# bioengstrom/tsbb15-3d-reconstruction-project

Measured on NVIDIA B200. Metric: f_ransac_evals_per_sec, higher is better.
Workload: dtype f32 scoring with f64 guard-band recheck; f64 solve

## Files before the change

include/rg_b200.h:

```cpp
#ifndef RG_B200_H
#define RG_B200_H

#include <stdint.h>

#ifdef __cplusplus
extern "C" {
#endif

#define RG_MODE_EPI_MAX 0
#define RG_MODE_SAMPSON 1
#define RG_TIE_FIRST 0
#define RG_TIE_REFERENCE 1
#define RG_SOLVER_QR 0
#define RG_SOLVER_JACOBI 1
#define RG_SCORE_FP32_GUARDED 0
#define RG_SCORE_FP64 1
#define RG_SCORE_FP32_BOUND 2

int rg_abi_version(void);
const char* rg_last_error(void);
int rg_init(int device, void** out_ctx);
int rg_shutdown(void* ctx);
int rg_device_sm_count(void* ctx);
int rg_host_alloc(size_t bytes, void** out);
int rg_host_free(void* p);
int rg_set_option(void* ctx, int option, long long value);
int rg_get_profile(void* ctx, void* stream, double* out_ms5, int* out_calls);

int rg_microbench_run(double* out6, void* stream);

int rg_get_last_stats(void* ctx, void* stream, long long* out8);

int rg_f_ransac_dev(void* ctx, void* stream, int P, const double* pts64_dev, const int32_t* pair_off_host,
                    const int32_t* idx_dev, const int32_t* hyp_off_host, double thr, int mode, int tie_mode, int solver,
                    int score_path, int32_t* best_idx_dev, int32_t* best_count_dev, double* best_F_dev,
                    unsigned char* mask_dev );
#define RG_FLAG_REUSE_POINTS 1
#define RG_FLAG_BOUNDED 2
int rg_f_ransac_dev2(void* ctx, void* stream, int P, const double* pts64_dev, const int32_t* pair_off_host,
                     const int32_t* idx_dev , const int32_t* hyp_off_host, double thr, int mode,
                     int tie_mode, int solver, int score_path, int flags, unsigned long long sample_seed, int first_pair_id,
                     int hyp_index_base, int32_t* best_idx_dev, int32_t* best_count_dev, double* best_F_dev,
                     unsigned char* mask_dev , unsigned long long* key_dev );
int rg_sample_indices_dev(void* ctx, void* stream, int P, const int32_t* n_points_host, const int32_t* hyp_off_host, int k,
                          unsigned long long seed, int first_pair_id, int hyp_index_base, int32_t* idx_out_dev);
int rg_synth_two_view_dev(void* ctx, void* stream, int P, int first_pair_id, int N, const double* cams_host, int n_cams,
                          const double* bbox6_host, unsigned long long seed_base, double outlier_frac, double sigma_px,
                          double width, double height, double* pts_out_dev, int32_t* cam_pair_out_dev);
int rg_f_inlier_mask_dev(void* ctx, void* stream, int P, const double* pts64_dev, const int32_t* pair_off_host,
                         const double* F_dev, double thr, int mode, unsigned char* mask_dev);
int rg_f_last_hypotheses_dev(void* ctx, const int32_t** counts_dev, const double** F_all_dev,
                             const unsigned char** flags_dev);
int rg_f_last_bounded_stats(void* ctx, void* stream, long long* out4);
int rg_f_last_bounded_evals(void* ctx, void* stream, long long* out2);
int rg_f_ransac_host(void* ctx, void* stream, int P, const double* pts64, const int32_t* pair_off, const int32_t* idx,
                     const int32_t* hyp_off, double thr, int mode, int tie_mode, int solver, int score_path,
                     int32_t* best_idx, int32_t* best_count, double* best_F, unsigned char* mask, int32_t* counts,
                     double* F_all, unsigned char* flags);

int rg_f_ransac_host2(void* ctx, void* stream, int P, const double* pts64, const int32_t* pair_off,
                      const int32_t* idx , const int32_t* hyp_off, double thr, int mode, int tie_mode,
                      int solver, int score_path, unsigned long long sample_seed, int first_pair_id, int32_t* best_idx,
                      int32_t* best_count, double* best_F, unsigned char* mask, int32_t* counts, double* F_all,
                      unsigned char* flags);

int rg_f8pt_solve_host(void* ctx, void* stream, int N, const double* pts64, int H, const int32_t* idx, int solver,
                       double* F_all, unsigned char* flags );
int rg_epi_score_count_host(void* ctx, void* stream, int N, const double* pts64, int H, const double* F_all, double thr,
                            int mode, int score_path, int32_t* counts);
int rg_fmatrix_residuals_host(void* ctx, void* stream, const double* F9, int N, const double* x, const double* y,
// ... 91 lines not shown
```

tsbb15-3d-reconstruction-project_b200/_cabi.py:

```python
from __future__ import annotations

import ctypes as C
import os
import threading

import numpy as np

_HERE = os.path.dirname(os.path.abspath(__file__))
LIB_PATH = os.environ.get("RG_LIB", os.path.join(_HERE, "librg_b200.so"))

MODE_EPI_MAX, MODE_SAMPSON = 0, 1
TIE_FIRST, TIE_REFERENCE = 0, 1
SOLVER_QR, SOLVER_JACOBI = 0, 1
SCORE_FP32_GUARDED, SCORE_FP64, SCORE_FP32_BOUND = 0, 1, 2
TRI_OPTIMAL, TRI_LINEAR = 0, 1
FLAG_REUSE_POINTS = 1
FLAG_BOUNDED = 2

_vp = C.c_void_p
_i = C.c_int
_d = C.c_double
_pd = C.POINTER(C.c_double)
_pll = C.POINTER(C.c_longlong)

SIGNATURES = {
    "rg_abi_version": (_i, []),
    "rg_last_error": (C.c_char_p, []),
    "rg_init": (_i, [_i, C.POINTER(_vp)]),
    "rg_shutdown": (_i, [_vp]),
    "rg_device_sm_count": (_i, [_vp]),
    "rg_host_alloc": (_i, [C.c_size_t, C.POINTER(_vp)]),
    "rg_host_free": (_i, [_vp]),
    "rg_set_option": (_i, [_vp, _i, C.c_longlong]),
    "rg_get_profile": (_i, [_vp, _vp, _pd, C.POINTER(C.c_int)]),
    "rg_microbench_run": (_i, [_pd, _vp]),
    "rg_get_last_stats": (_i, [_vp, _vp, _pll]),
    "rg_f_ransac_dev": (_i, [_vp, _vp, _i, _vp, _vp, _vp, _vp, _d, _i, _i, _i, _i, _vp, _vp, _vp, _vp]),
    "rg_f_ransac_dev2": (_i, [_vp, _vp, _i, _vp, _vp, _vp, _vp, _d, _i, _i, _i, _i, _i, C.c_ulonglong, _i, _i, _vp, _vp, _vp, _vp, _vp]),
    "rg_f_ransac_host2": (_i, [_vp, _vp, _i, _vp, _vp, _vp, _vp, _d, _i, _i, _i, _i, C.c_ulonglong, _i, _vp, _vp, _vp, _vp, _vp, _vp, _vp]),
    "rg_sample_indices_dev": (_i, [_vp, _vp, _i, _vp, _vp, _i, C.c_ulonglong, _i, _i, _vp]),
    "rg_synth_two_view_dev": (_i, [_vp, _vp, _i, _i, _i, _vp, _i, _vp, C.c_ulonglong, _d, _d, _d, _d, _vp, _vp]),
    "rg_f_inlier_mask_dev": (_i, [_vp, _vp, _i, _vp, _vp, _vp, _d, _i, _vp]),
    "rg_pnp_ransac_batched_dev2": (_i, [_vp, _vp, _i, _vp, _vp, _vp, _vp, _vp, _vp, _i, _d, _i, _i, _vp, _vp, _vp, _vp, _vp]),
    "rg_p2p_create": (_i, [_vp, _i, _i, _vp]),
    "rg_p2p_connect": (_i, [_vp, _vp]),
    "rg_p2p_destroy": (_i, [_vp]),
    "rg_p2p_argmax_exchange": (_i, [_vp, _vp, _i, _vp, _vp, _i, _vp, _vp, _vp, _vp]),
    "rg_f_last_hypotheses_dev": (_i, [_vp, C.POINTER(_vp), C.POINTER(_vp), C.POINTER(_vp)]),
    "rg_f_last_bounded_stats": (_i, [_vp, _vp, _pll]),
    "rg_f_last_bounded_evals": (_i, [_vp, _vp, _pll]),
    "rg_f_ransac_host": (_i, [_vp, _vp, _i, _vp, _vp, _vp, _vp, _d, _i, _i, _i, _i, _vp, _vp, _vp, _vp, _vp, _vp, _vp]),
    "rg_f8pt_solve_host": (_i, [_vp, _vp, _i, _vp, _i, _vp, _i, _vp, _vp]),
    "rg_epi_score_count_host": (_i, [_vp, _vp, _i, _vp, _i, _vp, _d, _i, _i, _vp]),
    "rg_fmatrix_residuals_host": (_i, [_vp, _vp, _vp, _i, _vp, _vp, _vp]),
    "rg_fmatrix_stls_host": (_i, [_vp, _vp, _i, _vp, _vp, _vp]),
    "rg_pnp_ransac_host": (_i, [_vp, _vp, _i, _i, _vp, _vp, _i, _i, _vp, _d, _i, _vp, _vp, _vp, _vp, _vp, _vp, _vp, _vp]),
    "rg_pnp_ransac_dev": (_i, [_vp, _vp, _i, _i, _vp, _vp, _i, _i, _vp, _d, _i, _vp, _vp, _vp, _vp]),
    "rg_pnp_ransac_batched_host": (_i, [_vp, _vp, _i, _vp, _vp, _vp, _vp, _vp, _vp, _i, _d, _i, _vp, _vp, _vp, _vp, _vp, _vp, _vp]),
    "rg_pnp_ransac_batched_dev": (_i, [_vp, _vp, _i, _vp, _vp, _vp, _vp, _vp, _vp, _i, _d, _i, _vp, _vp, _vp, _vp]),
    "rg_pnp_minimize_host": (_i, [_vp, _vp, _i, _vp, _vp, _vp, _vp]),
    "rg_pnp_score_count_host": (_i, [_vp, _vp, _i, _vp, _vp, _i, _vp, _d, _i, _vp]),
    "rg_triangulate_host": (_i, [_vp, _vp, _i, _vp, _vp, _vp, _vp, _vp, _i, _vp]),
    "rg_triangulate_dev": (_i, [_vp, _vp, _i, _vp, _vp, _vp, _vp, _vp, _i, _vp]),
    "rg_fmatrix_from_cameras_host": (_i, [_vp, _vp, _i, _vp, _vp, _vp]),
    "rg_relative_pose_host": (_i, [_vp, _vp, _i, _vp, _vp, _i, _vp, _vp, _vp, _vp, _vp]),
    "rg_relative_pose_dev": (_i, [_vp, _vp, _i, _vp, _vp, _i, _vp, _vp, _vp, _vp, _vp]),
    "rg_camera_resectioning_host": (_i, [_vp, _vp, _i, _vp, _vp, _vp, _vp]),
# ... 123 lines not shown
```

tsbb15-3d-reconstruction-project_b200/build.py:

```python
import os
import subprocess
import sys

HERE = os.path.dirname(os.path.abspath(__file__))
CSRC = os.path.join(HERE, "csrc")
LIB = os.path.join(HERE, "librg_b200.so")
SOURCES = ["librg_b200.cu"]
HEADERS = ["ctx.cu", "f_api.cu", "pnp_api.cu", "geom_api.cu", "geom_kernels.cuh", "gs_api.cu", "gs_kernels.cuh", "ba_api.cu", "ba_kernels.cuh", "nccl_api.cu", "p2p_api.cu", "philox.cuh", "microbench.cu", "common.cuh", "score_core.cuh", "f_kernels.cuh", "jacobi.cuh", "pnp_kernels.cuh", "pnp_refine_api.cu", "pnp_refine_kernels.cuh", "tall.cuh", "plan.cuh", "bounded.cuh"]
NVCC_FLAGS = ["-gencode", "arch=compute_100a,code=sm_100a", "-lineinfo", "-O3", "-std=c++17",
              "-Xcompiler", "-fPIC", "-shared", "-Xptxas", "-v", "-ldl"]


def _stale() -> bool:
    if not os.path.isfile(LIB):
        return True
    t = os.path.getmtime(LIB)
    for f in SOURCES + HEADERS:
        p = os.path.join(CSRC, f)
        if os.path.isfile(p) and os.path.getmtime(p) > t:
            return True
    return os.path.getmtime(os.path.abspath(__file__)) > t


LIB_DEBUG = os.path.join(HERE, "librg_b200_debug.so")


def build_debug(force: bool = False) -> str:
    if not force and os.path.isfile(LIB_DEBUG) and os.path.getmtime(LIB_DEBUG) >= max(
            os.path.getmtime(os.path.join(CSRC, f)) for f in SOURCES + HEADERS if os.path.isfile(os.path.join(CSRC, f))):
        return LIB_DEBUG
    nvcc = os.environ.get("NVCC", "/usr/local/cuda/bin/nvcc")
    flags = [f for f in NVCC_FLAGS if f not in ("-Xptxas", "-v")]
    cmd = [nvcc] + flags + ["-DRG_DEBUG"] + [os.path.join(CSRC, f) for f in SOURCES] + ["-o", LIB_DEBUG]
    res = subprocess.run(cmd, capture_output=True, text=True)
    if res.returncode != 0:
        sys.stderr.write(res.stdout + res.stderr)
        raise RuntimeError("nvcc failed building librg_b200_debug.so")
    return LIB_DEBUG


def build(force: bool = False, verbose: bool = False) -> str:
    if not force and not _stale():
        return LIB
    nvcc = os.environ.get("NVCC", "/usr/local/cuda/bin/nvcc")
    srcs = [os.path.join(CSRC, f) for f in SOURCES if os.path.isfile(os.path.join(CSRC, f))]
    cmd = [nvcc] + NVCC_FLAGS + srcs + ["-o", LIB]
    res = subprocess.run(cmd, capture_output=True, text=True)
    if verbose or res.returncode != 0:
        sys.stderr.write(res.stdout + res.stderr)
    if res.returncode != 0:
        raise RuntimeError("nvcc failed building librg_b200.so")
    with open(os.path.join(HERE, "build_ptxas.log"), "w") as f:
        f.write(res.stdout + res.stderr)
    return LIB


if __name__ == "__main__":
    print(build(force="--force" in sys.argv, verbose=True))
    if "--debug" in sys.argv:
        print(build_debug(force="--force" in sys.argv))
```

tsbb15-3d-reconstruction-project_b200/csrc/common.cuh:

```cuda
#pragma once
#include <cuda_runtime.h>
#include <cstdint>
#include <cstddef>
#include <cstdio>
#include <cstring>
#include <cmath>
#include <vector>
#ifdef RG_DEBUG
#include <cassert>
#define RG_ASSERT(cond) assert(cond)
#else
#define RG_ASSERT(cond) ((void)0)
#endif

namespace rg {

enum : int {
    RG_OK = 0,
    RG_ERR_CUDA = -1,
    RG_ERR_ARG = -2,
    RG_ERR_NO_DEVICE = -3,
};

void set_error(const char* fmt, ...);

#define RG_CUDA(call)                                                                       \
    do {                                                                                    \
        cudaError_t _e = (call);                                                            \
        if (_e != cudaSuccess) {                                                            \
            ::rg::set_error("%s:%d: %s -> %s", __FILE__, __LINE__, #call, cudaGetErrorString(_e)); \
            return ::rg::RG_ERR_CUDA;                                                       \
        }                                                                                   \
    } while (0)

#define RG_CHECK_ARG(cond, msg)                                   \
    do {                                                          \
        if (!(cond)) {                                            \
            ::rg::set_error("invalid argument: %s", msg);         \
            return ::rg::RG_ERR_ARG;                              \
        }                                                         \
    } while (0)

enum : int { MODE_EPI_MAX = 0, MODE_SAMPSON = 1 };
enum : int { TIE_FIRST = 0, TIE_REFERENCE = 1 };
enum : int { SOLVER_QR = 0, SOLVER_JACOBI = 1 };
enum : int { SCORE_FP32_GUARDED = 0, SCORE_FP64 = 1, SCORE_FP32_BOUND = 2 };

struct __align__(16) Hyp32 {
    float f[9];
    float g[5];
    float G;
    float T;
};
static_assert(sizeof(Hyp32) == 64, "Hyp32 layout");

struct __align__(16) Pose32 {
    float p[12];
    float G;
    float pad0, pad1, pad2;
};
static_assert(sizeof(Pose32) == 64, "Pose32 layout");

constexpr int kSub = 8;

__device__ __forceinline__ int find_segment(const int* __restrict__ off, int P, int i) {
    int lo = 0, hi = P;
    while (hi - lo > 1) {
        int mid = (lo + hi) >> 1;
        if (off[mid] <= i) lo = mid; else hi = mid;
    }
    return lo;
}

__device__ __forceinline__ uint32_t smem_u32(const void* p) {
    return (uint32_t)__cvta_generic_to_shared(p);
}

__device__ __forceinline__ void mbar_init(uint64_t* bar, uint32_t count) {
    asm volatile("mbarrier.init.shared::cta.b64 [%0], %1;" ::"r"(smem_u32(bar)), "r"(count));
}
__device__ __forceinline__ void fence_mbar_init() {
    asm volatile("fence.mbarrier_init.release.cluster;" ::: "memory");
}
__device__ __forceinline__ void fence_proxy_async() {
    asm volatile("fence.proxy.async.shared::cta;" ::: "memory");
}
__device__ __forceinline__ void mbar_expect_tx(uint64_t* bar, uint32_t bytes) {
    asm volatile("mbarrier.arrive.expect_tx.shared::cta.b64 _, [%0], %1;" ::"r"(smem_u32(bar)), "r"(bytes)
                 : "memory");
}
__device__ __forceinline__ bool mbar_try_wait(uint64_t* bar, uint32_t parity) {
    uint32_t ok;
    asm volatile(
        "{\n"
        ".reg .pred p;\n"
        "mbarrier.try_wait.parity.shared::cta.b64 p, [%1], %2;\n"
        "selp.u32 %0, 1, 0, p;\n"
        "}\n"
        : "=r"(ok)
// ... 35 lines not shown
    double c1x, c1y, c2x, c2y;
    double thr, B;
    double band_scale;
    double pad;
};

struct FPlan {
    int P = 0;
    long long Ntot = 0, Htot = 0, N32tot = 0;
    int n_items = 0;
    int maxN = 0, maxH = 0;
    double evals = 0.0;
    bool bounded = false;
    bool bound_prefix = false;
    int K = 0;
    long long Ctot = 0;
    int n_items_c = 0, n_items_f = 0;
    double evals_c = 0.0, evals_f = 0.0;
};

struct Ctx {
    int device = 0;
    int sm_count = 0;
    Buffer pair_info, pair_frame, state, pts32, F64, hyp32, flags, flag_list, stats, best, tie_stats, bbox;
    Buffer bnd;
    int* counts_ptr = nullptr;
    unsigned char* ovf_ptr = nullptr;
    Buffer gen_idx;
    struct PassSet { Buffer pair_info, pair_frame, state, pts32, F64, hyp32, flags, flag_list, best, tie_stats, bnd; } spare[3];
    cudaStream_t tail_stream = nullptr;
    cudaEvent_t head_done[3] = {nullptr, nullptr, nullptr};
    cudaEvent_t score_done[3] = {nullptr, nullptr, nullptr};
    cudaEvent_t cand_done[3] = {nullptr, nullptr, nullptr};
    cudaEvent_t sweep_done[3] = {nullptr, nullptr, nullptr};
    cudaEvent_t tail_done[2] = {nullptr, nullptr};
    cudaEvent_t pipe_gate = nullptr;
    bool tail_pending[2] = {false, false};
    int tail_carve_max = -1;
    int ws_slot = 0;
    int opt_pipeline = 1;
    const void* prep_pts = nullptr; int prep_P = 0; long long prep_N = 0; double prep_thr = 0.0; unsigned long long prep_hash = 0;
    int last_passes = 0;
    double rate_evals_per_s = 0.0, rate_h2d_bytes_per_s = 0.0;
    cudaEvent_t rate_ev[4] = {nullptr, nullptr, nullptr, nullptr};
    bool pnp_rows_attr_set = false;
    int opt_pnp_solver = 0;
    long long opt_list_cap = 0;
    double opt_band_scale = 1.0;
    long long opt_pass_evals = 0;
    int opt_bounded = 1;
    int opt_rho_milli = 450;
    int opt_bounded_k = 512;
    int opt_bound_prefix = 1;
    bool last_bounded = false;
    long long bnd_host_evals = 0;
    long long bnd_bound_evals = 0;
    Buffer bnd_stats;
    void* p2p_local = nullptr; size_t p2p_bytes = 0; int p2p_rank = 0, p2p_world = 0; unsigned p2p_seq = 0;
    void* p2p_peer[16] = {nullptr};

    Buffer d_in_a, d_in_b, d_in_c;
    Buffer d_out_a, d_out_b, d_out_c, d_out_d;
    Buffer pose64, pose32, X32;
    Buffer geom;
    Buffer geom_ws;
    Buffer gs_ws;
    Buffer ba_ws;
    int opt_ba_cluster = 0;
    int opt_gs_multi = 0;
    int opt_ba_l2 = 0;
    Buffer pr_ws;
    int opt_pr_multi = 0;
    Buffer h_pr_flags;
    cudaEvent_t pr_iter_ev[2] = {nullptr, nullptr};
    Buffer h_ba_items;
    Buffer h_ba_flags;
    cudaEvent_t ba_iter_ev[2] = {nullptr, nullptr};
    bool ba_attr_set = false;
    Buffer h_stage[2], h_stats;
    cudaEvent_t staging_free[2] = {nullptr, nullptr};
    int stage_turn = 0;
    FPlan plan_cached; unsigned long long plan_hash = 0; const void* plan_table = nullptr; bool plan_valid = false;
    static constexpr int kMaxSlices = 8;
    cudaStream_t copy_stream = nullptr;
    std::vector<cudaEvent_t> pass_ready;
    std::vector<cudaEvent_t> pass_done;
    cudaStream_t d2h_stream = nullptr;
    cudaEvent_t d2h_done = nullptr;
    cudaEvent_t copy_gate = nullptr;
    int opt_host_slices = 0;
    bool accumulate_stats = false;
    long long last_stats[8] = {0, 0, 0, 0, 0, 0, 0, 0};
    int opt_profile = 0;
    static constexpr int kProfPhases = 5;
    static constexpr int kProfScoreStart = 6;
    static constexpr int kProfSweep = 7;
    static constexpr int kProfEvents = 11;
    static constexpr int kProfRing = 2048;
    cudaEvent_t* prof_ev = nullptr;
    int prof_cur = -1;
    int prof_calls = 0;
    bool prof_open = false;
    unsigned prof_masks[kProfRing] = {0};
};

int ensure_pinned(Buffer& b, size_t bytes);
// ... 10 lines not shown
```

tsbb15-3d-reconstruction-project_b200/csrc/ctx.cu:

```cuda
#include "common.cuh"
#include <cstdarg>
#include <mutex>

namespace rg {

static thread_local char g_err[1024] = "";

void set_error(const char* fmt, ...) {
    va_list ap;
    va_start(ap, fmt);
    vsnprintf(g_err, sizeof(g_err), fmt, ap);
    va_end(ap);
}

int ensure(Buffer& b, size_t bytes) {
    if (bytes <= b.cap) return RG_OK;
    size_t want = bytes + bytes / 4 + 256;
    if (b.ptr) {
        RG_CUDA(cudaFree(b.ptr));
        b.ptr = nullptr;
        b.cap = 0;
    }
    RG_CUDA(cudaMalloc(&b.ptr, want));
    b.cap = want;
// ... 182 lines not shown
        c->opt_ba_l2 = value != 0;
        return RG_OK;
    }
    if (option == 5) {
        c->opt_gs_multi = value != 0;
        return RG_OK;
    }
    if (option == 6) {
        if (value < 0) { set_error("invalid argument: option 6 (evaluations per pass) must be >= 0"); return RG_ERR_ARG; }
        c->opt_pass_evals = value;
        return RG_OK;
    }
    if (option == 7) {
        if (value != 0 && value != 1) { set_error("invalid argument: option 7 (PnP minimal solver) must be 0 or 1"); return RG_ERR_ARG; }
        c->opt_pnp_solver = (int)value;
        return RG_OK;
    }
    if (option == 9) {
        if (value < 1000 || value > 100000000ll) { set_error("invalid argument: option 9 (guard-band factor x 1000) must be in [1000, 1e8]"); return RG_ERR_ARG; }
        c->opt_band_scale = (double)value / 1000.0;
        c->prep_pts = nullptr;
        return RG_OK;
    }
    if (option == 10) {
        if (value != 0 && value != 1) { set_error("invalid argument: option 10 (pass pipelining) must be 0 or 1"); return RG_ERR_ARG; }
        c->opt_pipeline = (int)value;
        return RG_OK;
    }
    if (option == 11) {
        if (value != 0 && value != 1) { set_error("invalid argument: option 11 (PnP refinement path) must be 0 or 1"); return RG_ERR_ARG; }
        c->opt_pr_multi = (int)value;
        return RG_OK;
    }
    if (option == 12) {
        if (value != 0 && value != 1) { set_error("invalid argument: option 12 (bounded sweep) must be 0 or 1"); return RG_ERR_ARG; }
        c->opt_bounded = (int)value;
        return RG_OK;
    }
    if (option == 13) {
        if (value < 1 || value > 1000) { set_error("invalid argument: option 13 (prefix share x 1000) must be in [1, 1000]"); return RG_ERR_ARG; }
        c->opt_rho_milli = (int)value;
        return RG_OK;
    }
    if (option == 14) {
        if (value < 1 || value > 65536) { set_error("invalid argument: option 14 (candidates per pair) must be in [1, 65536]"); return RG_ERR_ARG; }
        c->opt_bounded_k = (int)value;
        return RG_OK;
    }
    if (option == 15) {
        if (value != 0 && value != 1) { set_error("invalid argument: option 15 (bound-only prefix stage) must be 0 or 1"); return RG_ERR_ARG; }
        c->opt_bound_prefix = (int)value;
        return RG_OK;
    }
    if (option == 8) {
        if (value < 0 || value > 1000000000ll) { set_error("invalid argument: option 8 (flag list capacity) must be in [0, 1e9]"); return RG_ERR_ARG; }
        c->opt_list_cap = value;
        return RG_OK;
    }
    set_error("invalid argument: unknown option %d", option);
    return RG_ERR_ARG;
}

int rg_get_profile(void* ctx, void* stream, double* out_ms5, int* out_calls) {
    RG_CHECK_ARG(ctx != nullptr && out_ms5 != nullptr && out_calls != nullptr, "null argument");
    Ctx* c = (Ctx*)ctx;
    RG_CUDA(cudaSetDevice(c->device));
    RG_CUDA(cudaStreamSynchronize((cudaStream_t)stream));
    for (int k = 0; k < Ctx::kProfPhases; ++k) out_ms5[k] = 0.0;
    *out_calls = c->prof_calls;
    int complete = 0;
    for (int call = 0; call < c->prof_calls; ++call) {
        const unsigned need = (1u << (Ctx::kProfPhases + 1)) - 1u;
        if ((c->prof_masks[call] & need) != need) continue;
        cudaEvent_t* e = c->prof_ev + call * Ctx::kProfEvents;
        const bool own_start = (c->prof_masks[call] >> Ctx::kProfScoreStart) & 1u;
        for (int k = 0; k < Ctx::kProfPhases; ++k) {
            float ms = 0.f;
            RG_CUDA(cudaEventElapsedTime(&ms, (k == 2 && own_start) ? e[Ctx::kProfScoreStart] : e[k], e[k + 1]));
            out_ms5[k] += ms;
        }
        for (int b = Ctx::kProfSweep; b + 1 < Ctx::kProfEvents; b += 2) {
            if (((c->prof_masks[call] >> b) & 3u) != 3u) continue;
            float ms = 0.f;
            RG_CUDA(cudaEventElapsedTime(&ms, e[b], e[b + 1]));
            out_ms5[2] += ms;
        }
        ++complete;
    }
    *out_calls = complete;
    c->prof_calls = 0;
    c->prof_open = false;
    c->prof_cur = -1;
    return RG_OK;
}

}
```

tsbb15-3d-reconstruction-project_b200/csrc/f_api.cu:

```cuda
#include "f_kernels.cuh"
#include "bounded.cuh"
#include "jacobi.cuh"
#include "philox.cuh"
#include "plan.cuh"
#include <algorithm>
#include <vector>

namespace rg {

enum : int { FLAG_REUSE_POINTS = 1, FLAG_BOUNDED = 2 };

constexpr double kDefaultPassEvals = 2.7e10;
constexpr long long kMaxPassHyp = 1ll << 22;

struct ScoreState {
    unsigned* bbox; int* counts; int* work; unsigned* list_n; unsigned char* ovf;
    size_t off_counts, bytes;
    int *c_work, *f_work, *f_items, *sfx_c, *sfx_f, *mark;
    unsigned *c_list_n, *f_list_n;
    unsigned char *ovf_c, *ovf_f;
};

int score_state_layout(Ctx* c, int P, long long Htot, int bbox_words, ScoreState& s, long long Ctot = -1) {
    const size_t H = (size_t)std::max<long long>(Htot, 1);
    const size_t bbox_bytes = (((size_t)std::max(P, 1) * bbox_words * 4) + 15) / 16 * 16;
    const size_t cnt_bytes = ((H + 2) * 4 + 15) / 16 * 16;
    const size_t ovf_bytes = (H + 15) / 16 * 16;
    const size_t C = (size_t)std::max<long long>(Ctot, 1);
    const size_t bnd_ints = Ctot >= 0 ? ((8 + C + H + (size_t)std::max(P, 1)) * 4 + 15) / 16 * 16 : 0;
    const size_t bnd_ovf = Ctot >= 0 ? (C + H + 15) / 16 * 16 : 0;
    s.off_counts = bbox_bytes;
    s.bytes = bbox_bytes + cnt_bytes + ovf_bytes + bnd_ints + bnd_ovf;
    int rc = ensure(c->state, s.bytes);
    if (rc) return rc;
    char* base = (char*)c->state.ptr;
    s.bbox = (unsigned*)base;
    s.counts = (int*)(base + bbox_bytes);
    s.work = s.counts + H;
    s.list_n = (unsigned*)(s.counts + H + 1);
    s.ovf = (unsigned char*)(base + bbox_bytes + cnt_bytes);
    if (Ctot >= 0) {
        int* b = (int*)(base + bbox_bytes + cnt_bytes + ovf_bytes);
        s.c_work = b; s.c_list_n = (unsigned*)(b + 1); s.f_work = b + 2; s.f_list_n = (unsigned*)(b + 3); s.f_items = b + 4;
        s.sfx_c = b + 8; s.sfx_f = s.sfx_c + C; s.mark = s.sfx_f + H;
        s.ovf_c = (unsigned char*)(base + bbox_bytes + cnt_bytes + ovf_bytes + bnd_ints);
        s.ovf_f = s.ovf_c + C;
    }
    c->counts_ptr = s.counts;
    c->ovf_ptr = s.ovf;
    return RG_OK;
}

struct BndWs { Hyp32* hypc; int* map; int4* sel; PairInfo* fb; };
static int bnd_workspace(Ctx* c, const FPlan& plan, BndWs& w) {
// ... 137 lines not shown

template <int MODE>
static int f_solve_launch(Ctx* c, cudaStream_t st, const FPlan& plan, const double* pts64, const int* idx, int solver,
                          unsigned long long seed = 0, unsigned first_pair = 0) {
    const PairInfo* pi = (const PairInfo*)c->pair_info.ptr;
    const PairFrame* fr = (const PairFrame*)c->pair_frame.ptr;
    if (plan.Htot == 0) return RG_OK;
    if (solver == SOLVER_QR) {
        f8_solve_qr<MODE><<<ceil_div(plan.Htot, 128), 128, 0, st>>>((const double4*)pts64, idx, seed, first_pair, pi, fr, plan.P,
                                                                  (int)plan.Htot, (double*)c->F64.ptr, (Hyp32*)c->hyp32.ptr,
                                                                  (unsigned char*)c->flags.ptr);
    } else {
        const int groups_per_block = kJacobiThreads / 16;
        f8_solve_jacobi<MODE><<<ceil_div(plan.Htot, groups_per_block), kJacobiThreads, 0, st>>>(
            (const double4*)pts64, idx, seed, first_pair, pi, fr, plan.P, (int)plan.Htot, (double*)c->F64.ptr,
            (Hyp32*)c->hyp32.ptr, (unsigned char*)c->flags.ptr);
    }
    c->last_stats[7] += 1;
    RG_CUDA(cudaGetLastError());
    return RG_OK;
}

struct PassCtl {
    FCall a;
    std::vector<int> po, ho;
    FPlan plan;
    ScoreState s;
    FlagList fl{nullptr, nullptr, 0u, nullptr};
    FlagList flc{nullptr, nullptr, 0u, nullptr}, flf{nullptr, nullptr, 0u, nullptr};
    BndWs bw{};
    bool scored = false;
    int slot = 0;
    int prof_call = -1;
    cudaEvent_t ready = nullptr;
    cudaEvent_t done = nullptr;
    cudaStream_t out_stream = nullptr; void* out_dst = nullptr; const void* out_src = nullptr; size_t out_bytes = 0;
};

template <int MODE>
static int f_score_only(Ctx* c, cudaStream_t st, PassCtl& k) {
    const FPlan& plan = k.plan;
    const PairInfo* pi = (const PairInfo*)c->pair_info.ptr;
    k.scored = false;
    if (plan.Htot == 0 || plan.Ntot == 0 || (k.a.score_path != SCORE_FP64 && plan.n_items == 0)) return RG_OK;
    if (k.a.score_path != SCORE_FP64) {
        int bps = 1, rc = score_blocks_per_sm<EpiPolicy<MODE>>(&bps);
        if (rc) return rc;
        k.fl = flag_list_for(c, k.s, std::max(plan.evals, plan.evals_f), &rc);
        if (rc) return rc;
        if (plan.bounded) {
            k.flc = FlagList{k.fl.rec, k.s.c_list_n, k.fl.cap, k.s.ovf_c};
            k.flf = FlagList{k.fl.rec, k.s.f_list_n, k.fl.cap, k.s.ovf_f};
        }
        if (plan.bound_prefix || k.a.score_path == SCORE_FP32_BOUND) {
            static_assert(score_smem_bytes<EpiBoundPolicy>() == score_smem_bytes<EpiPolicy<MODE>>(), "same stage ring");
            if ((rc = score_blocks_per_sm<EpiBoundPolicy>(&bps))) return rc;
            score_packed<EpiBoundPolicy><<<std::min(plan.n_items, c->sm_count * bps), kScoreThreads,
                                           score_smem_bytes<EpiBoundPolicy>(), st>>>(
                (const float4*)c->pts32.ptr, (const Hyp32*)c->hyp32.ptr, pi, plan.P, plan.n_items, k.s.counts, k.fl, k.s.work);
        } else {
            constexpr size_t smem = score_smem_bytes<EpiPolicy<MODE>>();
            const int grid = std::min(plan.n_items, c->sm_count * bps);
            score_packed<EpiPolicy<MODE>><<<grid, kScoreThreads, smem, st>>>((const float4*)c->pts32.ptr, (const Hyp32*)c->hyp32.ptr,
                                                                            pi, plan.P, plan.n_items, k.s.counts, k.fl, k.s.work);
        }
        k.scored = true;
    } else {
        const int zs = std::max(1, std::min(64, ceil_div(plan.maxN, 2048)));
        f_score_fp64<<<dim3(ceil_div(plan.maxH, 128), plan.P, zs), 128, 0, st>>>((const double4*)k.a.pts64, (const double*)c->F64.ptr,
                                                                                 pi, k.a.thr, MODE, k.s.counts);
    }
    c->last_stats[7] += 1;
    RG_CUDA(cudaGetLastError());
    return RG_OK;
}

enum : int { STAGE_MAIN = 0, STAGE_CAND = 1, STAGE_FALLBACK = 2 };
template <int MODE>
static int f_fixup_launch(Ctx* c, cudaStream_t ts, PassCtl& k, bool beside_scorer, int stage = STAGE_MAIN) {
    if (!k.scored) return RG_OK;
    const FPlan& plan = k.plan;
    const PairInfo* pi = (const PairInfo*)c->pair_info.ptr;
    const Hyp32* hyp = (const Hyp32*)c->hyp32.ptr;
    const int* map = nullptr;
    FlagList fl = k.fl;
    long long H = plan.Htot;
    int* counts = k.s.counts;
    double evals = plan.evals;
    if (stage == STAGE_CAND) {
        pi += plan.P; hyp = k.bw.hypc; map = k.bw.map; fl = k.flc; H = plan.Ctot; counts = k.s.sfx_c; evals = plan.evals_c;
    } else if (stage == STAGE_FALLBACK) {
        pi = k.bw.fb; fl = k.flf; counts = k.s.sfx_f; evals = plan.evals_f;
    }
    typename EpiFix<MODE>::Params fp{(const float4*)c->pts32.ptr, (const double4*)k.a.pts64, hyp, (const double*)c->F64.ptr,
                                     pi, (const PairFrame*)c->pair_frame.ptr, plan.P, map};
    int fgrid = fixup_grid(c, evals);
    if (beside_scorer) {
        static const int forced = [] { const char* e = getenv("RG_TAIL_GRID"); return e ? atoi(e) : 0; }();
        fgrid = std::min(fgrid, forced > 0 ? forced : c->sm_count);
    }
    fixup_list<EpiFix<MODE>><<<fgrid, 256, 0, ts>>>(fp, fl, (int)H, counts, (unsigned long long*)c->stats.ptr);
    c->last_stats[7] += 1;
    RG_CUDA(cudaGetLastError());
    return RG_OK;
}

template <int MODE>
// ... 2 lines not shown
        int rc = k.plan.bound_prefix ? RG_OK : f_fixup_launch<MODE>(c, ts, k, beside_scorer);
        if (rc) return rc;
        const PairInfo* pi = (const PairInfo*)c->pair_info.ptr;
        bnd_select<<<k.plan.P, kSelectThreads, 0, ts>>>(k.s.counts, pi, pi + k.plan.P, (const Hyp32*)c->hyp32.ptr, k.bw.hypc,
                                                        k.bw.map, k.bw.sel);
        c->last_stats[7] += 1;
        RG_CUDA(cudaGetLastError());
    }
    prof_mark_at(c, ts, k.prof_call, 4);
    return RG_OK;
}

template <int MODE>
static int f_bnd_sweep(Ctx* c, cudaStream_t st, PassCtl& k) {
    if (!k.scored) return RG_OK;
    const FPlan& plan = k.plan;
    const PairInfo* pi = (const PairInfo*)c->pair_info.ptr;
    int bps = 1, rc = score_blocks_per_sm<EpiPolicy<MODE>>(&bps);
    if (rc) return rc;
    constexpr size_t smem = score_smem_bytes<EpiPolicy<MODE>>();
    prof_mark_at(c, st, k.prof_call, Ctx::kProfSweep);
    if (plan.n_items_c > 0) {
        score_packed<EpiPolicy<MODE>><<<std::min(plan.n_items_c, c->sm_count * bps), kScoreThreads, smem, st>>>(
            (const float4*)c->pts32.ptr, k.bw.hypc, pi + plan.P, plan.P, plan.n_items_c, k.s.sfx_c, k.flc, k.s.c_work);
        c->last_stats[7] += 1;
    }
    prof_mark_at(c, st, k.prof_call, Ctx::kProfSweep + 1);
    if (plan.n_items_c > 0 && (rc = f_fixup_launch<MODE>(c, st, k, false, STAGE_CAND))) return rc;
    bnd_check<<<plan.P, 256, 0, st>>>(k.s.counts, k.s.sfx_c, k.bw.map, pi, pi + plan.P, k.bw.sel, k.s.mark,
                                      (unsigned long long*)c->bnd_stats.ptr, !plan.bound_prefix);
    bnd_fb_plan<<<1, kSelectThreads, 0, st>>>(pi + 2 * (size_t)plan.P, k.s.mark, plan.P, k.bw.fb, k.s.f_items);
    c->last_stats[7] += 2;
    prof_mark_at(c, st, k.prof_call, Ctx::kProfSweep + 2);
    if (plan.n_items_f > 0) {
        score_packed<EpiPolicy<MODE>><<<std::min(plan.n_items_f, c->sm_count * bps), kScoreThreads, smem, st>>>(
            (const float4*)c->pts32.ptr, (const Hyp32*)c->hyp32.ptr, k.bw.fb, plan.P, plan.n_items_f, k.s.sfx_f, k.flf,
            k.s.f_work, k.s.f_items);
        c->last_stats[7] += 1;
    }
    prof_mark_at(c, st, k.prof_call, Ctx::kProfSweep + 3);
    RG_CUDA(cudaGetLastError());
    return RG_OK;
}

template <int MODE>
static int f_score_launch(Ctx* c, cudaStream_t st, const FPlan& plan, const ScoreState& s, const double* pts64, double thr,
                          int score_path) {
    PassCtl k;
    k.a.pts64 = pts64; k.a.thr = thr; k.a.score_path = score_path;
    k.plan = plan; k.s = s;
    int rc = f_score_only<MODE>(c, st, k);
    if (rc) return rc;
    prof_mark(c, st, 3);
    return score_path == SCORE_FP32_BOUND ? RG_OK : f_fixup_launch<MODE>(c, st, k, false);
}

static int f_select_launch(Ctx* c, cudaStream_t st, const FPlan& plan, const ScoreState& s, const double* pts64, double thr,
                           int mode, int tie_mode, unsigned char* mask, double* best_F, int* best_idx, int* best_count,
                           unsigned long long* keys) {
    if (plan.P == 0) return RG_OK;
    const PairInfo* pi = (const PairInfo*)c->pair_info.ptr;
    int2* best = (int2*)c->best.ptr;
    const bool tie = tie_mode == TIE_REFERENCE && plan.Htot > 0;
    if (!tie && mask == nullptr) {
        argmax_counts<<<plan.P, 256, 0, st>>>(s.counts, pi, best, (const unsigned char*)c->flags.ptr,
                                              (unsigned long long*)c->stats.ptr, keys, (const double*)c->F64.ptr, 9, best_F,
                                              best_idx, best_count);
        c->last_stats[7] += 1;
        RG_CUDA(cudaGetLastError());
        return RG_OK;
    }
    argmax_counts<<<plan.P, 256, 0, st>>>(s.counts, pi, best, (const unsigned char*)c->flags.ptr,
                                          (unsigned long long*)c->stats.ptr, tie ? nullptr : keys);
    c->last_stats[7] += 1;
    if (tie) {
        const int nb = (int)std::min<long long>(plan.Htot, (long long)c->sm_count * 8);
        f_tie_stats<<<nb, 256, 0, st>>>((const double4*)pts64, (const double*)c->F64.ptr, s.counts, pi, plan.P,
                                        (int)plan.Htot, best, mode, (double2*)c->tie_stats.ptr);
        f_tie_resolve<<<plan.P, 32, 0, st>>>(s.counts, pi, (const double2*)c->tie_stats.ptr, best, keys);
        c->last_stats[7] += 2;
    }
    const int nbx = mask ? std::max(1, std::min(64, ceil_div(plan.maxN, 256 * 4))) : 1;
    f_mask<<<dim3(nbx, plan.P), 256, 0, st>>>((const double4*)pts64, (const double*)c->F64.ptr, pi, best, thr, mode, mask, best_F,
                                              best_idx, best_count);
    c->last_stats[7] += 1;
    RG_CUDA(cudaGetLastError());
    return RG_OK;
}

static int f_pass_head(Ctx* c, cudaStream_t hs, PassCtl& k) {
    const FCall& a = k.a;
    FPlan& plan = k.plan;
    int bps = 1, rc = score_blocks_per_sm<EpiPolicy<MODE_EPI_MAX>>(&bps);
    if (rc) return rc;
    if ((rc = f_plan(c, hs, a.P, a.pair_off, a.hyp_off, plan, bps, nullptr, a.hyp_first, a.bounded ? c->opt_bounded_k : 0,
                     c->opt_rho_milli, a.bounded && c->opt_bound_prefix != 0)))
        return rc;
    for (int p = 0; p < a.P; ++p) {
        const int n = a.pair_off[p + 1] - a.pair_off[p], H = a.hyp_off[p + 1] - a.hyp_off[p];
        RG_CHECK_ARG(H == 0 || n >= 8, "a pair with hypotheses needs at least 8 correspondences");
    }
    const bool seeded = a.idx == nullptr && plan.Htot > 0;
    if ((rc = f_workspace(c, plan, seeded))) return rc;
    if ((rc = score_state_layout(c, a.P, plan.Htot, 8, k.s, a.bounded ? plan.Ctot : -1))) return rc;
    if (a.bounded && (rc = bnd_workspace(c, plan, k.bw))) return rc;
    if (a.P == 0) return RG_OK;
    if (plan.bound_prefix) {
// ... 649 lines not shown
        return rc;
    }
    if (piped) {
        if ((rc = pipe_join(c, st))) return rc;
        RG_CUDA(cudaMemcpyAsync(c->h_stats.ptr, c->stats.ptr, sizeof(unsigned long long) * 8, cudaMemcpyDeviceToHost, st));
    }
    if (stream_masks) {
        RG_CUDA(cudaEventRecord(c->d2h_done, c->d2h_stream));
        RG_CUDA(cudaStreamWaitEvent(st, c->d2h_done, 0));
    }
    RG_CUDA(cudaEventRecord(c->rate_ev[3], st));
    RG_CUDA(cudaMemcpyAsync(best_idx, d_idx, sizeof(int) * (size_t)P, cudaMemcpyDeviceToHost, st));
    RG_CUDA(cudaMemcpyAsync(best_count, d_cnt, sizeof(int) * (size_t)P, cudaMemcpyDeviceToHost, st));
    RG_CUDA(cudaMemcpyAsync(best_F, c->d_out_b.ptr, sizeof(double) * 9 * (size_t)P, cudaMemcpyDeviceToHost, st));
    if (mask && Ntot && !stream_masks) RG_CUDA(cudaMemcpyAsync(mask, c->d_out_c.ptr, Ntot, cudaMemcpyDeviceToHost, st));
    RG_CUDA(cudaStreamSynchronize(st));
    {
        float ms_up = 0.f, ms_run = 0.f;
        const double up_bytes = 32.0 * (double)Ntot + bytes_per_hyp * (double)Htot;
        double evals = 0.0;
        for (int p = 0; p < P; ++p) evals += (double)(pair_off[p + 1] - pair_off[p]) * (double)(hyp_off[p + 1] - hyp_off[p]);
        if (cudaEventElapsedTime(&ms_up, c->rate_ev[0], c->rate_ev[1]) == cudaSuccess && ms_up > 0.f && up_bytes > 1e6) {
            const double r = up_bytes / (ms_up * 1e-3);
            c->rate_h2d_bytes_per_s = c->rate_h2d_bytes_per_s > 0.0 ? 0.75 * c->rate_h2d_bytes_per_s + 0.25 * r : r;
        }
        if (cudaEventElapsedTime(&ms_run, c->rate_ev[2], c->rate_ev[3]) == cudaSuccess && ms_run > 0.f && evals > 1e9) {
            const double r = evals / (ms_run * 1e-3);
            c->rate_evals_per_s = c->rate_evals_per_s > 0.0 ? 0.75 * c->rate_evals_per_s + 0.25 * r : r;
        }
    }
    if (c->h_stats.ptr && ((const unsigned long long*)c->h_stats.ptr)[4] != 0) {
        set_error("invalid argument: %llu hypotheses have a sample index outside [0, N) of their pair",
                  ((const unsigned long long*)c->h_stats.ptr)[4]);
        return RG_ERR_ARG;
    }
    return RG_OK;
}

int rg_f_ransac_host(void* ctx, void* stream, int P, const double* pts64, const int* pair_off, const int* idx,
                     const int* hyp_off, double thr, int mode, int tie_mode, int solver, int score_path, int* best_idx,
                     int* best_count, double* best_F, unsigned char* mask, int* counts, double* F_all, unsigned char* flags) {
    RG_CHECK_ARG(P <= 0 || hyp_off == nullptr || hyp_off[P] == 0 || idx != nullptr,
                 "idx is null (use rg_f_ransac_host2 for device-drawn samples)");
    return rg_f_ransac_host2(ctx, stream, P, pts64, pair_off, idx, hyp_off, thr, mode, tie_mode, solver, score_path, 0ull, 0,
                             best_idx, best_count, best_F, mask, counts, F_all, flags);
}

int rg_epi_score_count_host(void* ctx, void* stream, int N, const double* pts64, int H, const double* F_all, double thr,
                            int mode, int score_path, int* counts) {
    RG_CHECK_ARG(ctx != nullptr, "ctx is null");
    RG_CHECK_ARG(N >= 0 && H >= 0 && counts, "bad sizes / null output");
    RG_CHECK_ARG(thr > 0.0 && std::isfinite(thr), "thr must be positive and finite");
    RG_CHECK_ARG(mode == MODE_EPI_MAX || mode == MODE_SAMPSON, "unknown scoring mode");
    RG_CHECK_ARG(score_path == SCORE_FP32_GUARDED || score_path == SCORE_FP64 || score_path == SCORE_FP32_BOUND,
                 "unknown scoring path");
    Ctx* c = (Ctx*)ctx;
    cudaStream_t st = (cudaStream_t)stream;
    RG_CUDA(cudaSetDevice(c->device));
    if (H == 0) return RG_OK;
    const int pair_off[2] = {0, N}, hyp_off[2] = {0, H};
    FPlan plan;
    int bps = 1, rc = score_blocks_per_sm<EpiPolicy<MODE_EPI_MAX>>(&bps);
    if (rc) return rc;
    if ((rc = f_plan(c, st, 1, pair_off, hyp_off, plan, bps))) return rc;
    if ((rc = f_workspace(c, plan, false))) return rc;
    ScoreState s;
    if ((rc = score_state_layout(c, 1, H, 8, s))) return rc;
    if ((rc = ensure(c->d_in_a, sizeof(double) * 4 * std::max<size_t>((size_t)N, 1)))) return rc;
    if (N) RG_CUDA(cudaMemcpyAsync(c->d_in_a.ptr, pts64, sizeof(double) * 4 * (size_t)N, cudaMemcpyHostToDevice, st));
    RG_CUDA(cudaMemcpyAsync(c->F64.ptr, F_all, sizeof(double) * 9 * (size_t)H, cudaMemcpyHostToDevice, st));
    c->last_stats[7] = 0;
    c->last_passes = 1;
    c->prep_pts = nullptr;
    RG_CUDA(cudaMemsetAsync(c->state.ptr, 0, s.bytes, st));
    RG_CUDA(cudaMemsetAsync(c->stats.ptr, 0, sizeof(unsigned long long) * 8, st));
    if ((rc = f_prepare(c, st, plan, s, (const double*)c->d_in_a.ptr, thr))) return rc;
    const PairInfo* pi = (const PairInfo*)c->pair_info.ptr;
    const PairFrame* fr = (const PairFrame*)c->pair_frame.ptr;
    if (mode == MODE_SAMPSON)
        f_make_hyp32<MODE_SAMPSON><<<ceil_div(H, 256), 256, 0, st>>>((const double*)c->F64.ptr, pi, fr, 1, H, (Hyp32*)c->hyp32.ptr);
    else
        f_make_hyp32<MODE_EPI_MAX><<<ceil_div(H, 256), 256, 0, st>>>((const double*)c->F64.ptr, pi, fr, 1, H, (Hyp32*)c->hyp32.ptr);
    c->last_stats[7] += 1;
    rc = (mode == MODE_SAMPSON) ? f_score_launch<MODE_SAMPSON>(c, st, plan, s, (const double*)c->d_in_a.ptr, thr, score_path)
                                : f_score_launch<MODE_EPI_MAX>(c, st, plan, s, (const double*)c->d_in_a.ptr, thr, score_path);
    if (rc) return rc;
    RG_CUDA(cudaMemcpyAsync(c->h_stats.ptr, c->stats.ptr, sizeof(unsigned long long) * 8, cudaMemcpyDeviceToHost, st));
    RG_CUDA(cudaMemcpyAsync(counts, s.counts, sizeof(int) * (size_t)H, cudaMemcpyDeviceToHost, st));
    RG_CUDA(cudaStreamSynchronize(st));
    return RG_OK;
}

int rg_f8pt_solve_host(void* ctx, void* stream, int N, const double* pts64, int H, const int* idx, int solver, double* F_all,
                       unsigned char* flags) {
    RG_CHECK_ARG(ctx != nullptr, "ctx is null");
    RG_CHECK_ARG(N >= 8 && H >= 0 && pts64 && F_all, "need N >= 8 and non-null buffers");
    RG_CHECK_ARG(solver == SOLVER_QR || solver == SOLVER_JACOBI, "unknown solver");
    Ctx* c = (Ctx*)ctx;
    cudaStream_t st = (cudaStream_t)stream;
    RG_CUDA(cudaSetDevice(c->device));
    if (H == 0) return RG_OK;
    RG_CHECK_ARG(idx != nullptr, "idx is null");
    const int pair_off[2] = {0, N}, hyp_off[2] = {0, H};
    FPlan plan;
    int bps = 1, rc = score_blocks_per_sm<EpiPolicy<MODE_EPI_MAX>>(&bps);
    if (rc) return rc;
    if ((rc = f_plan(c, st, 1, pair_off, hyp_off, plan, bps))) return rc;
// ... 45 lines not shown
```

Baseline: 5173 billion.

## Add tensor-core bound prefix scoring stage using split-fp16 MMA

Adds a new scoring kernel that evaluates the epipolar bound test with mma.sync fp16 tensor-core instructions. Point monomials and hypothesis entries are split into hi/lo fp16 parts, and a widened threshold keeps the test conservative. It is enabled by default for the bounded prefix path through a new option, replacing the scalar fp32 bound kernel there. The gain comes from tensor-core throughput, paid for with extra split and packing work and a looser bound that may pass more candidates on to later checks.

Result: faster. 5888 billion, median of 6 (+13.8%).

```diff
diff --git a/include/rg_b200.h b/include/rg_b200.h
--- a/include/rg_b200.h
+++ b/include/rg_b200.h
@@ -16,6 +16,7 @@
 #define RG_SCORE_FP32_GUARDED 0
 #define RG_SCORE_FP64 1
 #define RG_SCORE_FP32_BOUND 2
+#define RG_SCORE_TC_BOUND 3
 
 int rg_abi_version(void);
 const char* rg_last_error(void);
diff --git a/tsbb15-3d-reconstruction-project_b200/_cabi.py b/tsbb15-3d-reconstruction-project_b200/_cabi.py
--- a/tsbb15-3d-reconstruction-project_b200/_cabi.py
+++ b/tsbb15-3d-reconstruction-project_b200/_cabi.py
@@ -12,7 +12,7 @@
 MODE_EPI_MAX, MODE_SAMPSON = 0, 1
 TIE_FIRST, TIE_REFERENCE = 0, 1
 SOLVER_QR, SOLVER_JACOBI = 0, 1
-SCORE_FP32_GUARDED, SCORE_FP64, SCORE_FP32_BOUND = 0, 1, 2
+SCORE_FP32_GUARDED, SCORE_FP64, SCORE_FP32_BOUND, SCORE_TC_BOUND = 0, 1, 2, 3
 TRI_OPTIMAL, TRI_LINEAR = 0, 1
 FLAG_REUSE_POINTS = 1
 FLAG_BOUNDED = 2
diff --git a/tsbb15-3d-reconstruction-project_b200/build.py b/tsbb15-3d-reconstruction-project_b200/build.py
--- a/tsbb15-3d-reconstruction-project_b200/build.py
+++ b/tsbb15-3d-reconstruction-project_b200/build.py
@@ -6,7 +6,7 @@
 CSRC = os.path.join(HERE, "csrc")
 LIB = os.path.join(HERE, "librg_b200.so")
 SOURCES = ["librg_b200.cu"]
-HEADERS = ["ctx.cu", "f_api.cu", "pnp_api.cu", "geom_api.cu", "geom_kernels.cuh", "gs_api.cu", "gs_kernels.cuh", "ba_api.cu", "ba_kernels.cuh", "nccl_api.cu", "p2p_api.cu", "philox.cuh", "microbench.cu", "common.cuh", "score_core.cuh", "f_kernels.cuh", "jacobi.cuh", "pnp_kernels.cuh", "pnp_refine_api.cu", "pnp_refine_kernels.cuh", "tall.cuh", "plan.cuh", "bounded.cuh"]
+HEADERS = ["ctx.cu", "f_api.cu", "pnp_api.cu", "geom_api.cu", "geom_kernels.cuh", "gs_api.cu", "gs_kernels.cuh", "ba_api.cu", "ba_kernels.cuh", "nccl_api.cu", "p2p_api.cu", "philox.cuh", "microbench.cu", "common.cuh", "score_core.cuh", "f_kernels.cuh", "jacobi.cuh", "pnp_kernels.cuh", "pnp_refine_api.cu", "pnp_refine_kernels.cuh", "tall.cuh", "plan.cuh", "bounded.cuh", "tc_bound.cuh"]
 NVCC_FLAGS = ["-gencode", "arch=compute_100a,code=sm_100a", "-lineinfo", "-O3", "-std=c++17",
               "-Xcompiler", "-fPIC", "-shared", "-Xptxas", "-v", "-ldl"]
 
diff --git a/tsbb15-3d-reconstruction-project_b200/csrc/common.cuh b/tsbb15-3d-reconstruction-project_b200/csrc/common.cuh
--- a/tsbb15-3d-reconstruction-project_b200/csrc/common.cuh
+++ b/tsbb15-3d-reconstruction-project_b200/csrc/common.cuh
@@ -44,7 +44,7 @@
 enum : int { MODE_EPI_MAX = 0, MODE_SAMPSON = 1 };
 enum : int { TIE_FIRST = 0, TIE_REFERENCE = 1 };
 enum : int { SOLVER_QR = 0, SOLVER_JACOBI = 1 };
-enum : int { SCORE_FP32_GUARDED = 0, SCORE_FP64 = 1, SCORE_FP32_BOUND = 2 };
+enum : int { SCORE_FP32_GUARDED = 0, SCORE_FP64 = 1, SCORE_FP32_BOUND = 2, SCORE_TC_BOUND = 3 };
 
 struct __align__(16) Hyp32 {
     float f[9];
@@ -186,6 +186,7 @@
     int opt_rho_milli = 450;
     int opt_bounded_k = 512;
     int opt_bound_prefix = 1;
+    int opt_tc_bound = 1;
     bool last_bounded = false;
     long long bnd_host_evals = 0;
     long long bnd_bound_evals = 0;
diff --git a/tsbb15-3d-reconstruction-project_b200/csrc/ctx.cu b/tsbb15-3d-reconstruction-project_b200/csrc/ctx.cu
--- a/tsbb15-3d-reconstruction-project_b200/csrc/ctx.cu
+++ b/tsbb15-3d-reconstruction-project_b200/csrc/ctx.cu
@@ -258,6 +258,11 @@
         c->opt_bound_prefix = (int)value;
         return RG_OK;
     }
+    if (option == 16) {
+        if (value != 0 && value != 1) { set_error("invalid argument: option 16 (tensor-core prefix stage) must be 0 or 1"); return RG_ERR_ARG; }
+        c->opt_tc_bound = (int)value;
+        return RG_OK;
+    }
     if (option == 8) {
         if (value < 0 || value > 1000000000ll) { set_error("invalid argument: option 8 (flag list capacity) must be in [0, 1e9]"); return RG_ERR_ARG; }
         c->opt_list_cap = value;
diff --git a/tsbb15-3d-reconstruction-project_b200/csrc/f_api.cu b/tsbb15-3d-reconstruction-project_b200/csrc/f_api.cu
--- a/tsbb15-3d-reconstruction-project_b200/csrc/f_api.cu
+++ b/tsbb15-3d-reconstruction-project_b200/csrc/f_api.cu
@@ -1,5 +1,6 @@
 #include "f_kernels.cuh"
 #include "bounded.cuh"
+#include "tc_bound.cuh"
 #include "jacobi.cuh"
 #include "philox.cuh"
 #include "plan.cuh"
@@ -243,7 +244,17 @@
             k.flc = FlagList{k.fl.rec, k.s.c_list_n, k.fl.cap, k.s.ovf_c};
             k.flf = FlagList{k.fl.rec, k.s.f_list_n, k.fl.cap, k.s.ovf_f};
         }
-        if (plan.bound_prefix || k.a.score_path == SCORE_FP32_BOUND) {
+        const bool tc = k.a.score_path == SCORE_TC_BOUND || (plan.bound_prefix && c->opt_tc_bound != 0);
+        if (tc) {
+            static int tc_bps = 0;
+            if (tc_bps == 0) {
+                RG_CUDA(cudaOccupancyMaxActiveBlocksPerMultiprocessor(&tc_bps, score_tc_bound, kTcThreads, 0));
+                tc_bps = std::max(tc_bps, 1);
+            }
+            score_tc_bound<<<std::min(plan.n_items, c->sm_count * tc_bps), kTcThreads, 0, st>>>(
+                (const float4*)c->pts32.ptr, (const Hyp32*)c->hyp32.ptr, (const PairFrame*)c->pair_frame.ptr, pi, plan.P,
+                plan.n_items, k.s.counts, k.s.work);
+        } else if (plan.bound_prefix || k.a.score_path == SCORE_FP32_BOUND) {
             static_assert(score_smem_bytes<EpiBoundPolicy>() == score_smem_bytes<EpiPolicy<MODE>>(), "same stage ring");
             if ((rc = score_blocks_per_sm<EpiBoundPolicy>(&bps))) return rc;
             score_packed<EpiBoundPolicy><<<std::min(plan.n_items, c->sm_count * bps), kScoreThreads,
@@ -352,7 +363,7 @@
     int rc = f_score_only<MODE>(c, st, k);
     if (rc) return rc;
     prof_mark(c, st, 3);
-    return score_path == SCORE_FP32_BOUND ? RG_OK : f_fixup_launch<MODE>(c, st, k, false);
+    return (score_path == SCORE_FP32_BOUND || score_path == SCORE_TC_BOUND) ? RG_OK : f_fixup_launch<MODE>(c, st, k, false);
 }
 
 static int f_select_launch(Ctx* c, cudaStream_t st, const FPlan& plan, const ScoreState& s, const double* pts64, double thr,
@@ -1108,7 +1119,8 @@
     RG_CHECK_ARG(N >= 0 && H >= 0 && counts, "bad sizes / null output");
     RG_CHECK_ARG(thr > 0.0 && std::isfinite(thr), "thr must be positive and finite");
     RG_CHECK_ARG(mode == MODE_EPI_MAX || mode == MODE_SAMPSON, "unknown scoring mode");
-    RG_CHECK_ARG(score_path == SCORE_FP32_GUARDED || score_path == SCORE_FP64 || score_path == SCORE_FP32_BOUND,
+    RG_CHECK_ARG(score_path == SCORE_FP32_GUARDED || score_path == SCORE_FP64 || score_path == SCORE_FP32_BOUND ||
+                     score_path == SCORE_TC_BOUND,
                  "unknown scoring path");
     Ctx* c = (Ctx*)ctx;
     cudaStream_t st = (cudaStream_t)stream;
diff --git a/tsbb15-3d-reconstruction-project_b200/csrc/tc_bound.cuh b/tsbb15-3d-reconstruction-project_b200/csrc/tc_bound.cuh
--- /dev/null
+++ b/tsbb15-3d-reconstruction-project_b200/csrc/tc_bound.cuh
@@ -0,0 +1,181 @@
+#pragma once
+#include "score_core.cuh"
+#include <cuda_fp16.h>
+
+namespace rg {
+
+constexpr int kTcThreads = kHypPerBlock;
+constexpr int kTcTiles = kHypPerBlock / 16 / (kTcThreads / 32);
+constexpr int kTcChunk = 2 * kTcThreads;
+constexpr double kTcBoundE = 14.0 * 0x1p-22;
+static_assert(kTcTiles * 16 * (kTcThreads / 32) == kHypPerBlock, "one item = the warps' tiles");
+
+__host__ __device__ __forceinline__ float tc_bound_T(float T) {
+    const double a = sqrt((double)T) * 0.25 + kTcBoundE;
+#ifdef __CUDA_ARCH__
+    return __double2float_ru(a * a * (1.0 + 0x1p-40));
+#else
+    const double v = a * a * (1.0 + 0x1p-40);
+    float f = (float)v;
+    if ((double)f < v) f = nextafterf(f, INFINITY);
+    return f;
+#endif
+}
+
+__device__ __forceinline__ void tc_split(float v, float& hi, float& lo) {
+    hi = rintf(v * 2048.f) * 0x1p-11f;
+    lo = rintf((v - hi) * 0x1p21f) * 0x1p-21f;
+}
+__device__ __forceinline__ uint32_t h2u(float a, float b) {
+    const __half2 h = __floats2half2_rn(a, b);
+    return *reinterpret_cast<const uint32_t*>(&h);
+}
+
+__device__ __forceinline__ void tc_point(float x0, float x1, float y0, float y1, float ib, uint4& w0, uint4& w1) {
+    x0 *= ib; x1 *= ib; y0 *= ib; y1 *= ib;
+    const float m[8] = {x0 * y0, x0 * y1, x0, x1 * y0, x1 * y1, x1, y0, y1};
+    float hi[8], lo[8];
+#pragma unroll
+    for (int k = 0; k < 8; ++k) tc_split(m[k], hi[k], lo[k]);
+    w0 = make_uint4(h2u(hi[0], hi[1]), h2u(lo[0], lo[1]), h2u(hi[2], hi[3]), h2u(lo[2], lo[3]));
+    w1 = make_uint4(h2u(hi[4], hi[5]), h2u(lo[4], lo[5]), h2u(hi[6], hi[7]), h2u(lo[6], lo[7]));
+}
+
+__device__ __forceinline__ double tc_inv_bp(double B) {
+    int e;
+    const double fm = frexp(B, &e);
+    return ldexp(1.0, fm == 0.5 ? 1 - e : -e);
+}
+
+struct TcHyp {
+    uint32_t a1[2], a2[4];
+    float c1[4], c2[4], nT[2];
+};
+
+__device__ __forceinline__ void tc_load_hyp(const Hyp32* __restrict__ hyp32, int h0, int H_end, double bp, int g, int t, TcHyp& o) {
+    const float qnan = __int_as_float(0x7FFFFFFF);
+#pragma unroll
+    for (int r = 0; r < 2; ++r) {
+        const int h = h0 + g + 8 * r;
+        float f0 = qnan, f1 = qnan, f8 = qnan, T = 0.f;
+        if (h < H_end) {
+            const Hyp32& y = hyp32[h];
+            f0 = y.f[2 * t]; f1 = y.f[2 * t + 1]; f8 = y.f[8]; T = y.T;
+        }
+        const double s0 = (t == 1 || t == 3) ? bp : bp * bp;
+        const double s1 = (t == 0 || t == 1) ? bp * bp : bp;
+        float v0 = (float)((double)f0 * s0 * 0.25), v1 = (float)((double)f1 * s1 * 0.25), v8 = f8 * 0.25f;
+        const float Tp = tc_bound_T(T);
+        if (isinf(Tp)) { v0 = v1 = v8 = 0.f; }
+        float h0v, l0v, h1v, l1v, h8v, l8v;
+        tc_split(v0, h0v, l0v);
+        tc_split(v1, h1v, l1v);
+        tc_split(v8, h8v, l8v);
+        o.a1[r] = h2u(h0v, h1v);
+        o.a2[r] = h2u(l0v, l1v);
+        o.a2[2 + r] = o.a1[r];
+        o.c1[2 * r] = o.c1[2 * r + 1] = h8v;
+        o.c2[2 * r] = o.c2[2 * r + 1] = l8v;
+        o.nT[r] = -Tp;
+    }
+}
+
+__device__ __forceinline__ void mma_k8(float (&d)[4], const uint32_t (&a)[2], uint32_t b, const float (&c)[4]) {
+    asm("mma.sync.aligned.m16n8k8.row.col.f32.f16.f16.f32 {%0,%1,%2,%3}, {%4,%5}, {%6}, {%7,%8,%9,%10};"
+        : "=f"(d[0]), "=f"(d[1]), "=f"(d[2]), "=f"(d[3])
+        : "r"(a[0]), "r"(a[1]), "r"(b), "f"(c[0]), "f"(c[1]), "f"(c[2]), "f"(c[3]));
+}
+__device__ __forceinline__ void mma_k16(float (&d)[4], const uint32_t (&a)[4], uint32_t b0, uint32_t b1, const float (&c)[4]) {
+    asm("mma.sync.aligned.m16n8k16.row.col.f32.f16.f16.f32 {%0,%1,%2,%3}, {%4,%5,%6,%7}, {%8,%9}, {%10,%11,%12,%13};"
+        : "=f"(d[0]), "=f"(d[1]), "=f"(d[2]), "=f"(d[3])
+        : "r"(a[0]), "r"(a[1]), "r"(a[2]), "r"(a[3]), "r"(b0), "r"(b1), "f"(c[0]), "f"(c[1]), "f"(c[2]), "f"(c[3]));
+}
+
+__global__ void __maxnreg__(96)
+score_tc_bound(const float4* __restrict__ pts32, const Hyp32* __restrict__ hyp32, const PairFrame* __restrict__ frames,
+               const PairInfo* __restrict__ pi, int P, int n_items, int* __restrict__ counts, int* __restrict__ work_counter) {
+    __shared__ __align__(16) uint2 sb[2][kTcChunk * 4];
+    __shared__ int s_next;
+    const int tid = threadIdx.x, lane = tid & 31, warp = tid >> 5;
+    const int g = lane >> 2, t = lane & 3;
+    int item = blockIdx.x;
+    if (item >= n_items) return;
+    ScoreItem cur = decode_item(pi, P, item);
+    int buf = 0;
+    auto load_pair = [&](const ScoreItem& it, int done, float4& X, float4& Y) {
+        const int total = (it.g1 - it.g0) * kSub;
+        if (done + 2 * tid < total) {
+            const float4* src = pts32 + ((size_t)pi[it.pair].pt_off32 + (size_t)it.g0 * kSub + done) + 2 * (size_t)tid;
+            X = src[0]; Y = src[1];
+        }
+    };
+    float4 X = make_float4(0.f, 0.f, 0.f, 0.f), Y = X;
+    load_pair(cur, 0, X, Y);
+    while (true) {
+        if (tid == 0) s_next = (int)gridDim.x + atomicAdd(work_counter, 1);
+        const double ibd = tc_inv_bp(frames[cur.pair].B);
+        const float ib = (float)ibd;
+        TcHyp hy[kTcTiles];
+        unsigned cnt[kTcTiles][2];
+#pragma unroll
+        for (int j = 0; j < kTcTiles; ++j) {
+            tc_load_hyp(hyp32, cur.h_base + (warp * kTcTiles + j) * 16, cur.H_end, 1.0 / ibd, g, t, hy[j]);
+            cnt[j][0] = cnt[j][1] = 0u;
+        }
+        __syncthreads();
+        const int next_item = s_next;
+        const bool has_next = next_item < n_items;
+        ScoreItem nxt = cur;
+        if (has_next) nxt = decode_item(pi, P, next_item);
+        const int total = (cur.g1 - cur.g0) * kSub;
+        for (int done = 0; done < total; done += kTcChunk) {
+            const int npts = min(total - done, kTcChunk);
+            if (2 * tid < npts) {
+                uint4 w0, w1, w2, w3;
+                tc_point(X.x, X.z, Y.x, Y.z, ib, w0, w1);
+                tc_point(X.y, X.w, Y.y, Y.w, ib, w2, w3);
+                uint4* dst = reinterpret_cast<uint4*>(&sb[buf][0]);
+                const int n = 2 * tid;
+                const int base = ((n >> 3) * 32 + (n & 7) * 4) / 2;
+                dst[base] = w0; dst[base + 1] = w1; dst[base + 2] = w2; dst[base + 3] = w3;
+            }
+            __syncthreads();
+            if (done + kTcChunk < total) load_pair(cur, done + kTcChunk, X, Y);
+            else if (has_next) load_pair(nxt, 0, X, Y);
+            const uint2* sp = &sb[buf][0];
+#pragma unroll 1
+            for (int c8 = 0; c8 < npts / 8; ++c8) {
+                const uint2 b = sp[c8 * 32 + lane];
+#pragma unroll
+                for (int j = 0; j < kTcTiles; ++j) {
+                    float d1[4], d2[4];
+                    mma_k8(d1, hy[j].a1, b.x, hy[j].c1);
+                    mma_k16(d2, hy[j].a2, b.x, b.y, hy[j].c2);
+#pragma unroll
+                    for (int r = 0; r < 2; ++r) {
+                        const float2 rr = __fadd2_rn(make_float2(d1[2 * r], d1[2 * r + 1]), make_float2(d2[2 * r], d2[2 * r + 1]));
+                        const float2 qq = __ffma2_rn(rr, rr, make_float2(hy[j].nT[r], hy[j].nT[r]));
+                        cnt[j][r] += __float_as_uint(qq.x) >> 31;
+                        cnt[j][r] += __float_as_uint(qq.y) >> 31;
+                    }
+                }
+            }
+            buf ^= 1;
+        }
+#pragma unroll
+        for (int j = 0; j < kTcTiles; ++j)
+#pragma unroll
+            for (int r = 0; r < 2; ++r) {
+                unsigned v = cnt[j][r];
+                v += __shfl_xor_sync(0xffffffffu, v, 1);
+                v += __shfl_xor_sync(0xffffffffu, v, 2);
+                const int h = cur.h_base + (warp * kTcTiles + j) * 16 + g + 8 * r;
+                if (t == 0 && h < cur.H_end && v) atomicAdd(&counts[h], (int)v);
+            }
+        if (!has_next) break;
+        __syncthreads();
+        cur = nxt;
+    }
+}
+
+}
```
